# pkhungurn/talking-head-anime-4-demo

Hardware: NVIDIA H100
Metric: 512x512 RGBA frames/sec (higher is better)
Workload: dtype f16/tf32 operands (10-bit mantissa), f32 accumulate, f32 storage outside conv operands

## Files before the change

tha4_b200/csrc/capi.cu:

```cuda
#include "../../include/tha4_b200.h"
#include "nets.cuh"
#include "siren.cuh"
#include "profiler.cuh"
#include "distill.cuh"
#include <atomic>
#include <cstring>
#include <map>
#include <tuple>
#include <vector>

namespace tha4 {
std::atomic<long> g_kernel_launches{0};
bool g_use_pdl = true;
thread_local AllocSink* g_alloc_sink = nullptr;
void* tracked_malloc(size_t bytes) {
    void* p = nullptr;
    THA4_CUDA_CHECK(cudaMalloc(&p, std::max<size_t>(bytes, 16)));
    if (g_alloc_sink) g_alloc_sink->ptrs.push_back(p);
    return p;
}
}

using namespace tha4;

// ... 206 lines not shown
    if (ctx->capture_stream) cudaStreamDestroy(ctx->capture_stream);
    if (ctx->side) { cudaStreamDestroy(ctx->side); cudaEventDestroy(ctx->ev_fork); cudaEventDestroy(ctx->ev_join); }
    if (ctx->stats_base) cudaFree(ctx->stats_base);
    ctx->drop_graphs();
    delete ctx;
    return THA4_OK;
}

const char* tha4_last_error(const tha4_ctx* ctx) { return ctx ? ctx->err.c_str() : g_create_err.c_str(); }

int tha4_set_option(tha4_ctx* ctx, const char* name, int64_t value) {
    return guarded(ctx, [&] {
        cudaDeviceSynchronize();
        ctx->drop_graphs();
        if (!strcmp(name, "strict")) { ctx->strict = value ? 1 : 0; }
        else if (!strcmp(name, "cuda_graphs")) ctx->use_graphs = value ? 1 : 0;
        else if (!strcmp(name, "side_stream")) ctx->side_streams = value ? 1 : 0;
        else if (!strcmp(name, "tcgen05")) conv_enable_tc(value != 0);
        else if (!strcmp(name, "cluster_splitk")) conv_tc_enable_cluster(value != 0);
        else if (!strcmp(name, "halo_conv")) conv_halo_enable(value != 0);
        else if (!strcmp(name, "tma_store")) conv_halo_enable_tma_store(value != 0);
        else if (!strcmp(name, "halo_m256")) { THA4_REQUIRE(value >= -1 && value <= 1, "halo_m256: -1, 0 or 1"); conv_halo_set_m256((int)value); }
        else if (!strcmp(name, "halo_ctas")) { THA4_REQUIRE(value == -1 || value == 1 || value == 2, "halo_ctas: -1, 1 or 2"); conv_halo_set_ctas((int)value); }
        else if (!strcmp(name, "siren_tc")) siren_tc_enable(value != 0);
        else if (!strcmp(name, "tc_stride2")) conv_tc_enable_stride2(value != 0);
        else if (!strcmp(name, "small_bn")) conv_tc_enable_small_bn(value != 0);
        else if (!strcmp(name, "attn_split16")) attention_enable_split16(value != 0);
        else if (!strcmp(name, "tail_persist")) tail_tc_enable_persist(value != 0);
        else if (!strcmp(name, "attn_mma")) attention_enable_mma(value != 0);
        else if (!strcmp(name, "half_operands")) ctx->half_operands = value ? 1 : 0;
        else if (!strcmp(name, "pdl")) g_use_pdl = value != 0;
        else if (!strcmp(name, "profile")) { prof_enable(value != 0); if (value == 2) prof_reset(); }
        else if (!strcmp(name, "microbatch")) { THA4_REQUIRE(value >= 1 && value <= 1024, "microbatch range"); ctx->microbatch = (int)value; }
        else throw std::runtime_error(std::string("tha4: unknown option ") + name);
    });
}

int64_t tha4_get_counter(const tha4_ctx* ctx, const char* name) {
    if (!strcmp(name, "kernel_launches")) return g_kernel_launches.load();
    {
        static const char* cats[] = {"conv", "norm", "tail", "attn", "glue", "siren"};
        static const char* whats[] = {"us", "launches", "flops", "bytes"};
        if (!strncmp(name, "prof_", 5))
            for (int w = 0; w < 4; ++w)
                for (int c = 0; c < 6; ++c)
                    if (std::string(name) == std::string("prof_") + whats[w] + "_" + cats[c]) {
// ... 969 lines not shown
```

tha4_b200/csrc/conv.cuh:

```cuda
#pragma once
#include "common.cuh"

namespace tha4 {

constexpr int CONV_MAX_TAPS = 16;
constexpr int CONV_MAX_PHASES = 4;

enum ResMode { RES_NONE = 0, RES_SAME = 1, RES_UP2 = 2, RES_DOWN2 = 3 };

struct ConvWeights {
    float* w = nullptr;
    mutable __half* w16 = nullptr;
    mutable float w16_scale = 1.0f;
    float* bias = nullptr;
    int cin = 0, cout = 0, cin_pad = 0, cout_pad = 0;
    int ntaps = 0, nphase = 1;
    bool dynamic = false;
    bool tf32_rounded = false;
    int stride = 1;
    int out_mul = 1;
    signed char dy[CONV_MAX_PHASES][CONV_MAX_TAPS];
    signed char dx[CONV_MAX_PHASES][CONV_MAX_TAPS];
    signed char ph_oy[CONV_MAX_PHASES], ph_ox[CONV_MAX_PHASES];
};
// ... 24 lines not shown
    View out16;
    ConvNormIn nin;
    View res;
    int res_mode = RES_NONE;
    int strict = 0;
    int ksplit = 0;
    float* ws = nullptr;
    size_t ws_floats = 0;
};

size_t conv_workspace_floats(const ConvWeights& cw, const ConvArgs& a);

void conv_forward(const ConvWeights& cw, const ConvArgs& a, cudaStream_t s);
void conv_mma_forward(const ConvWeights& cw, const ConvArgs& a, cudaStream_t s);
bool conv_tc_supported(const ConvWeights& cw, const ConvArgs& a);
void conv_tc_forward(const ConvWeights& cw, const ConvArgs& a, cudaStream_t s);
bool conv_fuses_stats(const ConvWeights& cw, const ConvArgs& a);
bool conv_tc_fuses_stats(const ConvWeights& cw, const ConvArgs& a);
bool conv_halo_supported(const ConvWeights& cw, const ConvArgs& a);
void conv_halo_forward(const ConvWeights& cw, const ConvArgs& a, cudaStream_t s);
void conv_halo_enable(bool on);
void conv_halo_enable_tma_store(bool on);
void conv_halo_set_ctas(int mode);
void conv_halo_set_m256(int mode);
void conv_halo_debug_dump();
void conv_enable_tc(bool on);
bool conv_tc_enabled();
void conv_make_half(const ConvWeights& cw, cudaStream_t s);
void conv_tc_enable_cluster(bool on);
void conv_tc_enable_small_bn(bool on);
void conv_tc_enable_stride2(bool on);

}
```

tha4_b200/csrc/conv_halo.cu:

```cuda
#include "conv.cuh"
#include "profiler.cuh"
#include "conv_tc_device.cuh"
#include <cuda.h>
#include <cstring>
#include <map>
#include <mutex>
#include <tuple>

namespace tha4 {
static long long* g_dbg_buf = nullptr;

namespace {

using namespace tc;
using namespace tcdev;

constexpr int HT_W = 8, HT_H = 16;
constexpr int HALO_W = HT_W + 2;
__host__ __device__ constexpr int halo_h(int wg) { return HT_H * wg + 2; }
__host__ __device__ constexpr int halo_rows(int wg) { return HALO_W * halo_h(wg); }
__host__ __device__ constexpr int halo_a_bytes(int rowb, int wg) { return ((halo_rows(wg) * rowb + 1023) / 1024) * 1024; }
__host__ __device__ constexpr int halo_threads(int wg, int ctas = 1) { return 128 * wg + (ctas == 2 ? 0 : 32); }
static_assert((HT_H * HALO_W * 64) % 1024 == 0, "second warpgroup's halo offset keeps the swizzle phase");

__host__ __device__ constexpr int halo_min_ctas(int bn, int sa, int cs, int op, int wg, int ph = 1, int ctas = 1) {
    return ctas == 2 ? 2 : wg > 1 ? (bn * (ph == 4 ? 2 : 1) <= 32 ? 2 : 1) : cs > 1 || bn >= 128 ? 1 : ((sa == (op == OP_F16N ? 2 : 1) && bn <= 32) ? 4 : 2);
}
template <int PH>
__host__ __device__ constexpr int halo_wtile(int j) { return PH == 1 ? j : ((j & 1) * 2 + ((j >> 1) & 1)) * 4 + (j >> 2); }

template <int BN, int SA, int SB, int CS, int OP, int XF, int WG, int PH = 1, int CTAS = 1>
__global__ void __launch_bounds__(halo_threads(WG, CTAS), halo_min_ctas(BN, SA, CS, OP, WG, PH, CTAS)) conv_halo_kernel(const __grid_constant__ CUtensorMap tmA, const __grid_constant__ CUtensorMap tmB,
                                                                const __grid_constant__ CUtensorMap tmO32, const __grid_constant__ CUtensorMap tmO16,
                                                                const __grid_constant__ CUtensorMap tmR, const TcParams p) {
    static_assert(OP != OP_TF32, "halo kernel: f16 operands");
    static_assert(BN <= 128, "the accumulator of one warpgroup: BN registers per thread");
    static_assert(WG == 1 || (WG == 2 && CS == 1 && BN <= 64), "two consumer warpgroups: unsplit launches, two accumulators of at most 64 columns");
    static_assert(PH == 1 || (PH == 4 && WG == 2 && BN <= 32), "four-phase layers: two warpgroups, two 128 x 32 accumulators each");
    constexpr bool SELF_LOAD = CTAS == 2;
    static_assert(CTAS == 1 || (CTAS == 2 && WG == 2), "two CTAs per SM: the two-warpgroup tiles");
    static_assert(!SELF_LOAD || SB >= (PH == 1 ? 3 : 6), "weight ring too shallow for loads issued by a consumer");
    constexpr int SLABS = PH == 1 ? WG : 1;
    constexpr int NACC = PH == 1 ? 1 : 2;
    constexpr int TPC = PH == 1 ? 9 : 16;
    constexpr int ROWB = op_row_bytes(OP);
    constexpr int KCE = op_kch(OP);
    constexpr int HALO_ROWS = halo_rows(SLABS);
    constexpr int A_BYTES = halo_a_bytes(ROWB, SLABS);
    constexpr int B_BYTES = BN * ROWB;
    constexpr int PRODUCER_WARP = 4 * WG;
    constexpr int EPI_BYTES = (int)(((size_t)SA * A_BYTES + (size_t)SB * B_BYTES) / WG) & ~1023;
    constexpr int NSLOT = CS == 1 && PH == 1 ? epi_nslot(BN, EPI_BYTES) : 0;
    extern __shared__ uint8_t smem_raw[];
    uint8_t* smem = smem_raw + ((1024u - (tc::smem_u32(smem_raw) & 1023u)) & 1023u);
    uint8_t* smA = smem;
    uint8_t* smB = smem + SA * A_BYTES;
    uint64_t* bars = reinterpret_cast<uint64_t*>(smB + SB * B_BYTES);
    uint64_t* a_full = bars, *a_empty = bars + SA;
    uint64_t* b_full = bars + 2 * SA, *b_empty = b_full + SB;
    uint64_t* res_bars = b_empty + SB;
    float* xf_A = reinterpret_cast<float*>(reinterpret_cast<uint8_t*>(res_bars + 4 * WG) + ((16u - (tc::smem_u32(res_bars + 4 * WG) & 15u)) & 15u));

    const int warp = threadIdx.x >> 5, lane = threadIdx.x & 31;
    auto dbg_slot = [&]() -> long long* {
        const bool dbg_on = p.dbg != nullptr && (blockIdx.x % 97) == 0 && blockIdx.y == 0 && (blockIdx.x / 97) * CS + blockIdx.z < 32;
        return dbg_on ? p.dbg + ((blockIdx.x / 97) * CS + blockIdx.z) * 32 : nullptr;
    };
    long long* dbg = SELF_LOAD ? nullptr : dbg_slot();
#define HSTAMP(role, i) do { long long* d_ = SELF_LOAD ? dbg_slot() : dbg; if (d_) d_[(role) * 8 + (i)] = clock64(); } while (0)
#define HSTAMP_END(role, i) do { if (!SELF_LOAD) HSTAMP(role, i); } while (0)
    if (threadIdx.x == 0) HSTAMP(0, 0);
    int tile = blockIdx.x;
    const int tx = tile % p.tiles_x; tile /= p.tiles_x;
    const int ty = tile % p.tiles_y;
    const int n = tile / p.tiles_y;
// ... 25 lines not shown
        }
    }
    pdl_wait();
    if (threadIdx.x == 0) HSTAMP(0, 2);

    Acc<BN> acc[NACC];
    if (nc > 0) {
        if (!SELF_LOAD && warp == PRODUCER_WARP) {
            if (lane == 0) {
                int bi = 0;
                for (int ci = 0; ci < nc; ++ci) {
                    const int sa = ci % SA;
                    mbar_wait(smem_u32(a_empty + sa), ((ci / SA) & 1) ^ 1);
                    mbar_expect_tx(smem_u32(a_full + sa), HALO_ROWS * ROWB);
                    tma_load_4d(smem_u32(smA + sa * A_BYTES), &tmA, (cb0 + ci) * KCE, x0 - 1, y0 - 1, n, smem_u32(a_full + sa));
                    for (int tap = 0; tap < TPC; ++tap, ++bi) {
                        if (bi < npre) continue;
                        const int sb = bi % SB;
                        mbar_wait(smem_u32(b_empty + sb), ((bi / SB) & 1) ^ 1);
                        mbar_expect_tx(smem_u32(b_full + sb), B_BYTES);
                        tma_load_3d(smem_u32(smB + sb * B_BYTES), &tmB, (cb0 + ci) * KCE, n0, halo_wtile<PH>(tap), smem_u32(b_full + sb));
                    }
                }
            }
        } else {
            const int te = threadIdx.x;
            const int wg = WG == 1 ? 0 : te >> 7;
            constexpr int XBAR = WG == 1 ? 1 : 3;
            __half* hA = reinterpret_cast<__half*>(xf_A);
            __half* hB = hA + p.xf_C;
            const bool silu = p.xf_act == ACT_SILU || p.xf_act == ACT_SILU_FAST;
            auto load_b = [&](int j) {
                if (j < SB || j >= nb) return;
                const int sb = j % SB;
                mbar_wait(smem_u32(b_empty + sb), ((j / SB) & 1) ^ 1);
                mbar_expect_tx(smem_u32(b_full + sb), B_BYTES);
                tma_load_3d(smem_u32(smB + sb * B_BYTES), &tmB, (cb0 + j / TPC) * KCE, n0, halo_wtile<PH>(j % TPC), smem_u32(b_full + sb));
            };
            auto load_a = [&](int ci) {
                if (ci >= nc) return;
                const int sa = ci % SA;
                mbar_wait(smem_u32(a_empty + sa), ((ci / SA) & 1) ^ 1);
                mbar_expect_tx(smem_u32(a_full + sa), HALO_ROWS * ROWB);
                tma_load_4d(smem_u32(smA + sa * A_BYTES), &tmA, (cb0 + ci) * KCE, x0 - 1, y0 - 1, n, smem_u32(a_full + sa));
            };
            if (SELF_LOAD && te == 0) {
// ... 79 lines not shown
                            Wgmma<BN>::f16(acc[0].d[0], make_desc_sbo<ROWB>(a0 + 32 * k, HALO_W * ROWB), bd, accum);
                            Wgmma<BN>::f16(acc[0].d[1], make_desc_sbo<ROWB>(a1 + 32 * k, HALO_W * ROWB), bd, accum);
                        }
                        wg_commit();
                        if (tap < 8) {
                            wg_wait<1>();
                            if (tap > 0) mbar_arrive(smem_u32(b_empty + (bi - 1) % SB));
                        } else {
                            wg_wait<0>();
                            mbar_arrive(smem_u32(b_empty + (bi - 1) % SB));
                            mbar_arrive(smem_u32(b_empty + bi % SB));
                            mbar_arrive(smem_u32(a_empty + sa));
                        }
                        if (SELF_LOAD && te == 0) {
                            load_b(bi + SB - 2);
                            if (tap == 8) load_a(ci + SA);
                        }
                    }
                }
            }
#pragma unroll
            for (int a = 0; a < NACC; ++a) { wg_fence_acc(acc[a].d[0]); wg_fence_acc(acc[a].d[1]); }
            if (te == 0) { HSTAMP_END(1, 1); HSTAMP_END(2, 3); }
            if constexpr (WG > 1) asm volatile("bar.sync 3, 256;\n" ::: "memory");
            if constexpr (PH == 4) {
#pragma unroll
                for (int px = 0; px < 2; ++px) {
                    if (px > 0) asm volatile("bar.sync 3, 256;\n" ::: "memory");
                    epi_direct<BN, HT_W, 0, WG>(p, acc[px], smem + wg * EPI_BYTES, n, y0, x0, n0, 2 * wg + px, 0, warp, lane,
                                                nullptr, nullptr, nullptr, nullptr, wg, EPI_BYTES);
                }
            } else if (CS == 1) {
                epi_direct<BN, HT_W, NSLOT, WG>(p, acc[0], smem + wg * EPI_BYTES, n, y0 + wg * HT_H, x0, n0, 0, 0, warp, lane,
                                                &tmO32, &tmO16, &tmR, res_bars + 4 * wg, wg, EPI_BYTES);
            }
            if (te == 0) HSTAMP_END(2, 4);
        }
    }
    if (CS > 1) {
        asm volatile("barrier.cluster.arrive.release.aligned;\n" ::: "memory");
        asm volatile("barrier.cluster.wait.acquire.aligned;\n" ::: "memory");
        if (threadIdx.x == 0) HSTAMP(2, 5);
        if (warp < PRODUCER_WARP && nc > 0) epi_push_partial<BN, CS>(acc[0], smem, split, warp, lane);
        asm volatile("barrier.cluster.arrive.release.aligned;\n" ::: "memory");
        asm volatile("barrier.cluster.wait.acquire.aligned;\n" ::: "memory");
        if (threadIdx.x == 0) HSTAMP(2, 7);
        if (warp < PRODUCER_WARP) epi_cluster_reduce<BN, CS, HT_W>(p, smem, n, y0, x0, n0, 0, split, warp, dbg);
        if (threadIdx.x == 0) HSTAMP(2, 6);
    }
    __syncthreads();
    if (threadIdx.x == 0) HSTAMP_END(0, 3);
#undef HSTAMP_END
#undef HSTAMP
}

typedef CUresult (*EncodeTiledFn)(CUtensorMap*, CUtensorMapDataType, cuuint32_t, void*, const cuuint64_t*, const cuuint64_t*,
                                  const cuuint32_t*, const cuuint32_t*, CUtensorMapInterleave, CUtensorMapSwizzle,
                                  CUtensorMapL2promotion, CUtensorMapFloatOOBfill);
EncodeTiledFn halo_encode() {
    static EncodeTiledFn fn = nullptr;
    if (!fn) {
        void* ptr = nullptr;
// ... 47 lines not shown
    const int es = f16 ? 2 : 4;
    if (!v.p || (reinterpret_cast<uintptr_t>(v.p) & 15) || ((long)v.ld * es) % 16 != 0) return false;
    HKey key{current_device(), v.p, v.N, v.H, v.W, v.C, v.ld, f16 ? -2 : -3};
    std::lock_guard<std::mutex> lock(g_halo_mu);
    auto it = g_halo_maps.find(key);
    if (it == g_halo_maps.end()) {
        CUtensorMap m;
        cuuint64_t dims[4] = {(cuuint64_t)v.C, (cuuint64_t)v.W, (cuuint64_t)v.H, (cuuint64_t)v.N};
        cuuint64_t strides[3] = {(cuuint64_t)v.ld * es, (cuuint64_t)v.W * v.ld * es, (cuuint64_t)v.H * v.W * v.ld * es};
        cuuint32_t box[4] = {32, (cuuint32_t)HT_W, (cuuint32_t)HT_H, 1};
        cuuint32_t estr[4] = {1, 1, 1, 1};
        CUresult r = halo_encode()(&m, f16 ? CU_TENSOR_MAP_DATA_TYPE_FLOAT16 : CU_TENSOR_MAP_DATA_TYPE_FLOAT32, 4, v.p, dims, strides, box, estr,
                                   CU_TENSOR_MAP_INTERLEAVE_NONE, f16 ? CU_TENSOR_MAP_SWIZZLE_64B : CU_TENSOR_MAP_SWIZZLE_128B,
                                   CU_TENSOR_MAP_L2_PROMOTION_NONE, CU_TENSOR_MAP_FLOAT_OOB_FILL_NONE);
        if (r != CUDA_SUCCESS) return false;
        it = g_halo_maps.emplace(key, m).first;
    }
    *out = &it->second;
    return true;
}

int g_halo_m256 = -1;
int g_halo_ctas = -1;

constexpr size_t halo_ring(int op, int bn, int sa, int sb, int wg, int ph) {
    return (size_t)sa * halo_a_bytes(op_row_bytes(op), ph == 1 ? wg : 1) + (size_t)sb * bn * op_row_bytes(op);
}
constexpr size_t halo_smem0(int op, int bn, int sa, int sb, int wg, int ph) {
    return 1024 + halo_ring(op, bn, sa, sb, wg, ph) + (2 * sa + 2 * sb + 4 * wg) * 8 + 16;
}

struct HaloPlan { int bn, tiles_x, tiles_y, tiles_m, tiles_n, cs, chunks, wg, ctas; };

constexpr int halo_sb_wg2(int op, int bn, int sa, int sb_min) {
    const size_t a = (size_t)sa * halo_a_bytes(op_row_bytes(op), 2), b = (size_t)bn * op_row_bytes(op);
    int sb = sb_min;
    while (a + sb * b < 2 * (size_t)(epi_slot0(bn) + EPI_SLOT_BYTES)) ++sb;
    return sb;
}
constexpr int halo2_sa(int op, int ph) { return ph == 4 || op == OP_F16N ? 2 : 1; }
constexpr int halo2_sb(int op, int ph) { return ph == 4 ? 12 : halo_sb_wg2(op, 64, halo2_sa(op, ph), op == OP_F16N ? 12 : 6); }

int halo_plan_ctas(int op, int bn, int ph, long ctas, const ConvArgs& a) {
    if (g_halo_ctas > 0) return g_halo_ctas;
    const size_t smem = halo_smem0(op, bn, halo2_sa(op, ph), halo2_sb(op, ph), 2, ph) + (a.nin.on ? (size_t)24 * a.nin.C + 32 : 0);
    return ctas > num_sms() && 2 * (smem + 1024) <= (size_t)228 * 1024 ? 2 : 1;
}

HaloPlan halo_plan(const ConvWeights& cw, const ConvArgs& a, int op) {
    HaloPlan pl;
    pl.chunks = cw.cin_pad / op_kch(op);
    if (cw.nphase == 4) {
        pl.tiles_x = ceil_div(a.in.W, HT_W); pl.tiles_y = ceil_div(a.in.H, HT_H);
        pl.tiles_m = pl.tiles_x * pl.tiles_y * a.in.N;
        pl.bn = 32; pl.tiles_n = cw.cout_pad / 32; pl.cs = 1; pl.wg = 2;
        pl.ctas = halo_plan_ctas(op, 32, 4, (long)pl.tiles_m * pl.tiles_n, a);
        return pl;
    }
    pl.tiles_x = ceil_div(a.out.W, HT_W); pl.tiles_y = ceil_div(a.out.H, HT_H);
    pl.tiles_m = pl.tiles_x * pl.tiles_y * a.in.N;
    pl.bn = (cw.cout_pad % 128 == 0) ? 128 : (cw.cout_pad % 64 == 0 ? 64 : 32);
    const int sms = num_sms();
    pl.cs = 1;
    long ctas = (long)pl.tiles_m * (cw.cout_pad / pl.bn);
    const bool m256 = g_halo_m256 > 0 || (g_halo_m256 < 0 && a.ksplit <= 1 && 8L * pl.tiles_m >= sms);
    if (a.ksplit > 1) {
        while (pl.cs * 2 <= std::min(8, a.ksplit)) pl.cs *= 2;
    } else if (a.ksplit <= 0 && ctas < sms * 13 / 16 && !m256) {
        while (pl.bn > 64 && (long)pl.tiles_m * (cw.cout_pad / pl.bn) < sms && cw.cout_pad % (pl.bn / 2) == 0) pl.bn /= 2;
        ctas = (long)pl.tiles_m * (cw.cout_pad / pl.bn);
        const int want = std::max(2, (int)((3 * sms / 2 + ctas - 1) / ctas));
        while (pl.cs < 8 && pl.cs * 2 <= want && pl.cs * 2 <= pl.chunks) pl.cs *= 2;
        while (pl.bn > 32 && (long)pl.tiles_m * (cw.cout_pad / pl.bn) * pl.cs < 96 && cw.cout_pad % (pl.bn / 2) == 0) pl.bn /= 2;
    }
    while (pl.cs > 1 && (pl.cs > pl.chunks || ceil_div(pl.chunks, ceil_div(pl.chunks, pl.cs)) != pl.cs)) pl.cs /= 2;
    pl.tiles_n = cw.cout_pad / pl.bn;
    pl.wg = 1;
    if (pl.cs == 1 && m256) {
        pl.wg = 2;
        pl.tiles_y = ceil_div(a.out.H, 2 * HT_H);
        pl.tiles_m = pl.tiles_x * pl.tiles_y * a.in.N;
        pl.bn = std::min(pl.bn, 64);
        pl.tiles_n = cw.cout_pad / pl.bn;
    }
    pl.ctas = pl.wg == 2 && pl.bn == 64 ? halo_plan_ctas(op, 64, 1, (long)pl.tiles_m * pl.tiles_n, a) : 1;
    return pl;
}

template <int OP, int BN, int SA, int SB, int CS, int XF, int WG = 1, int PH = 1, int CTAS = 1>
void launch_halo(const CUtensorMap& ma, const CUtensorMap& mb, const CUtensorMap& mo32, const CUtensorMap& mo16, const CUtensorMap& mr, const TcParams& p, dim3 grid, cudaStream_t s) {
    constexpr size_t ring = halo_ring(OP, BN, SA, SB, WG, PH);
    constexpr size_t smem0 = halo_smem0(OP, BN, SA, SB, WG, PH);
    static_assert(smem0 <= 227 * 1024, "shared memory budget");
    static_assert(ring / WG >= (size_t)4 * 32 * 33 * 4 + 4 * BN * 8, "epilogue scratch must fit in the pipeline buffers");
    static_assert(WG == 1 || PH == 4 || epi_nslot(BN, (ring / WG) & ~(size_t)1023) > 0, "two warpgroups: a TMA-store staging slot each");
    static_assert(CS == 1 || ring >= (size_t)128 * BN * 4 + 128 * 8 * 4 + 128 * 4 * 4, "partial tile + statistics scratch must fit");
    static_assert(CTAS == 1 || 2 * (smem0 + 1024) <= 228 * 1024, "two CTAs per SM");
    const size_t smem = smem0 + (XF ? (size_t)24 * p.xf_C + 32 : 0);
    THA4_REQUIRE(smem <= 227 * 1024, "conv_halo: shared memory budget (fused input normalisation)");
    THA4_ENSURE_SMEM((conv_halo_kernel<BN, SA, SB, CS, OP, XF, WG, PH, CTAS>), smem);
    launch_pdl(conv_halo_kernel<BN, SA, SB, CS, OP, XF, WG, PH, CTAS>, grid, dim3(halo_threads(WG, CTAS)), smem, s, CS, ma, mb, mo32, mo16, mr, p);
    THA4_LAUNCH_CHECK();
}

template <int OP, int BN, int SA, int SBD, int SBS, int XF>
void launch_halo_cs(int cs, int wg, int ctas, const CUtensorMap& ma, const CUtensorMap& mb, const CUtensorMap& mo32, const CUtensorMap& mo16, const CUtensorMap& mr, const TcParams& p, dim3 grid, cudaStream_t s) {
    constexpr int SA1 = OP == OP_F16N ? 2 : 1;
    THA4_REQUIRE(wg == 1 || (BN <= 64 && cs == 1), "conv_halo: 256-pixel tiles need an unsplit launch with N tiles of at most 64 columns");
    THA4_REQUIRE(ctas == 1 || (wg == 2 && BN == 64), "conv_halo: two CTAs per SM are built for 256 x 64 tiles");
    if constexpr (BN == 64) {
        if (ctas == 2) {
            launch_halo<OP, 64, halo2_sa(OP, 1), halo2_sb(OP, 1), 1, XF, 2, 1, 2>(ma, mb, mo32, mo16, mr, p, grid, s);
            return;
        }
    }
    if constexpr (BN <= 64) {
        if (cs == 1 && p.cpt == 1) {
            if (wg == 2) launch_halo<OP, BN, SA1, halo_sb_wg2(OP, BN, SA1, BN == 64 ? SBD : SBS), 1, XF, 2>(ma, mb, mo32, mo16, mr, p, grid, s);
            else launch_halo<OP, BN, SA1, SBS, 1, XF>(ma, mb, mo32, mo16, mr, p, grid, s);
            return;
        }
    }
    if constexpr (BN <= 64) {
        if (wg == 2) {
            constexpr int M = OP == OP_F16N ? 2 : 1;
            launch_halo<OP, BN, SA, halo_sb_wg2(OP, BN, SA, BN == 64 ? SBD : 2 * M), 1, XF, 2>(ma, mb, mo32, mo16, mr, p, grid, s);
            return;
        }
    }
    if (cs == 8) launch_halo<OP, BN, SA, SBD, 8, XF>(ma, mb, mo32, mo16, mr, p, grid, s);
    else if (cs == 4) launch_halo<OP, BN, SA, SBD, 4, XF>(ma, mb, mo32, mo16, mr, p, grid, s);
    else if (cs == 2) launch_halo<OP, BN, SA, SBD, 2, XF>(ma, mb, mo32, mo16, mr, p, grid, s);
    else if ((long)grid.x * grid.y * grid.z <= num_sms())
        launch_halo<OP, BN, SA, SBD, 1, XF>(ma, mb, mo32, mo16, mr, p, grid, s);
    else launch_halo<OP, BN, SA, SBS, 1, XF>(ma, mb, mo32, mo16, mr, p, grid, s);
}

template <int OP, int XF>
void launch_halo_bn(int bn, int cs, int wg, int ctas, const CUtensorMap& ma, const CUtensorMap& mb, const CUtensorMap& mo32, const CUtensorMap& mo16, const CUtensorMap& mr, const TcParams& p, dim3 grid, cudaStream_t s) {
    constexpr int M = OP == OP_F16N ? 2 : 1;
    if (bn == 128) launch_halo_cs<OP, 128, 2 * M, 6 * M, 3 * M, XF>(cs, wg, ctas, ma, mb, mo32, mo16, mr, p, grid, s);
    else if (bn == 64) launch_halo_cs<OP, 64, 2 * M, 8 * M, 3 * M, XF>(cs, wg, ctas, ma, mb, mo32, mo16, mr, p, grid, s);
    else launch_halo_cs<OP, 32, 2 * M, 9 * M, 5 * M, XF>(cs, wg, ctas, ma, mb, mo32, mo16, mr, p, grid, s);
}

bool g_use_halo = true;
bool g_tma_store = true;

}

void conv_halo_enable(bool on) { g_use_halo = on; }
void conv_halo_enable_tma_store(bool on) { g_tma_store = on; }
void conv_halo_set_m256(int mode) { g_halo_m256 = mode; }
void conv_halo_set_ctas(int mode) { g_halo_ctas = mode; }

bool conv_halo_supported(const ConvWeights& cw, const ConvArgs& a) {
    if (!g_use_halo || !conv_tc_supported(cw, a)) return false;
    if (!a.in.f16 || cw.stride != 1) return false;
    const bool four_phase = cw.nphase == 4 && cw.ntaps == 4 && cw.out_mul == 2;
    if (!four_phase && (cw.ntaps != 9 || cw.nphase != 1 || cw.out_mul != 1)) return false;
    for (int ph = 0; ph < cw.nphase; ++ph)
        for (int t = 0; t < cw.ntaps; ++t)
            if (cw.dy[ph][t] < -1 || cw.dy[ph][t] > 1 || cw.dx[ph][t] < -1 || cw.dx[ph][t] > 1) return false;
    if (!four_phase) return a.in.H == a.out.H && a.in.W == a.out.W;
    if (cw.cin_pad % 64 != 0 || a.ksplit > 1 || a.out.H != 2 * a.in.H || a.out.W != 2 * a.in.W) return false;
    const HaloPlan pl = halo_plan(cw, a, OP_F16);
    return a.ksplit == 1 || (long)pl.tiles_m * pl.tiles_n >= 64;
}

bool conv_halo_fuses_stats(const ConvWeights&, const ConvArgs&) { return true; }

void conv_halo_forward(const ConvWeights& cw, const ConvArgs& a, cudaStream_t s) {
    THA4_REQUIRE(conv_halo_supported(cw, a), "conv_halo: unsupported configuration");
    THA4_REQUIRE(a.in.C == cw.cin && a.out.C == cw.cout && a.in.N == a.out.N, "conv_halo: shapes");
    const int op = cw.cin_pad % 64 == 0 ? OP_F16 : OP_F16N;
    TcParams p{};
    p.out = a.out.p; p.outH = a.out.H; p.outW = a.out.W; p.outC = a.out.C; p.out_ld = a.out.ld;
// ... 22 lines not shown
    p.acc_scale = 1.0f / cw.w16_scale;
    for (int ph = 0; ph < cw.nphase; ++ph) {
        p.ph_oy[ph] = cw.ph_oy[ph]; p.ph_ox[ph] = cw.ph_ox[ph];
        for (int t = 0; t < cw.ntaps; ++t) { p.dy[ph][t] = cw.dy[ph][t]; p.dx[ph][t] = cw.dx[ph][t]; }
    }
    p.ksplit = 1;
    p.ws = nullptr;
    p.stats = a.out.stats; p.stats_ld = a.out.stats_ld;
    p.stats_rep = std::max(1, a.out.stats_rep); p.stats_rep_stride = a.out.stats_rep_stride;
    static const bool dbg_env = getenv("THA4_HALO_DEBUG") != nullptr;
    if (dbg_env) {
        if (!g_dbg_buf) { THA4_CUDA_CHECK(cudaMalloc(&g_dbg_buf, 32 * 32 * sizeof(long long))); }
        THA4_CUDA_CHECK(cudaMemsetAsync(g_dbg_buf, 0, 32 * 32 * sizeof(long long), s));
        p.dbg = g_dbg_buf;
    }
    ProfScope prof(PROF_CONV, s);
    prof_add_work(PROF_CONV, 2.0 * (double)p.N * p.MH * p.MW * cw.cout * cw.cin * cw.ntaps * cw.nphase, 0.0);
    const CUtensorMap& ma = halo_activation_map(a.in, op, cw.nphase == 1 ? pl.wg : 1);
    const CUtensorMap& mb = halo_weight_map(cw, pl.bn, op);
    const CUtensorMap* mo32 = &ma;
    const CUtensorMap* mo16 = &ma;
    const CUtensorMap* mr = &ma;
    p.st_tma = 0;
    if (pl.cs == 1 && g_tma_store && cw.nphase == 1) {
        if (a.out.p && halo_store_map(a.out, false, &mo32)) p.st_tma |= 1;
        if (a.out16.p && halo_store_map(a.out16, true, &mo16)) p.st_tma |= 2;
        if ((p.st_tma & 1) && a.res.p && p.res_mode == RES_SAME && !a.res.f16 && a.res.N == a.out.N && a.res.H == a.out.H &&
            a.res.W == a.out.W && a.res.C >= a.out.C && halo_store_map(a.res, false, &mr)) p.st_tma |= 4;
    }
    p.vec4 = ((!cw.bias || (reinterpret_cast<uintptr_t>(cw.bias) & 15) == 0) &&
              (!a.res.p || ((reinterpret_cast<uintptr_t>(a.res.p) & 15) == 0 && a.res.ld % 4 == 0))) ? 1 : 0;
    dim3 grid(pl.tiles_m, pl.tiles_n, pl.cs);
    if (cw.nphase == 4) {
        constexpr int SA2 = halo2_sa(OP_F16, 4), SB2 = halo2_sb(OP_F16, 4);
        if (pl.ctas == 2) {
            if (a.nin.on) launch_halo<OP_F16, 32, SA2, SB2, 1, 1, 2, 4, 2>(ma, mb, *mo32, *mo16, *mr, p, grid, s);
            else launch_halo<OP_F16, 32, SA2, SB2, 1, 0, 2, 4, 2>(ma, mb, *mo32, *mo16, *mr, p, grid, s);
        } else if (a.nin.on) launch_halo<OP_F16, 32, 2, 16, 1, 1, 2, 4>(ma, mb, *mo32, *mo16, *mr, p, grid, s);
        else launch_halo<OP_F16, 32, 2, 16, 1, 0, 2, 4>(ma, mb, *mo32, *mo16, *mr, p, grid, s);
    } else if (op == OP_F16) {
        if (a.nin.on) launch_halo_bn<OP_F16, 1>(pl.bn, pl.cs, pl.wg, pl.ctas, ma, mb, *mo32, *mo16, *mr, p, grid, s);
        else launch_halo_bn<OP_F16, 0>(pl.bn, pl.cs, pl.wg, pl.ctas, ma, mb, *mo32, *mo16, *mr, p, grid, s);
    } else {
        if (a.nin.on) launch_halo_bn<OP_F16N, 1>(pl.bn, pl.cs, pl.wg, pl.ctas, ma, mb, *mo32, *mo16, *mr, p, grid, s);
        else launch_halo_bn<OP_F16N, 0>(pl.bn, pl.cs, pl.wg, pl.ctas, ma, mb, *mo32, *mo16, *mr, p, grid, s);
    }
    static const bool dbg_all = dbg_env && !strcmp(getenv("THA4_HALO_DEBUG"), "2");
    if (dbg_all) {
        fprintf(stderr, "halo launch: N %d %dx%d cin %d cout %d | bn %d cs %d wg %d chunks %d grid %d x %d | xf %d groups %d act %d res %d out32 %d out16 %d st_tma %d | phases %d ctas %d\n",
                p.N, p.MH, p.MW, cw.cin, cw.cout, pl.bn, pl.cs, pl.wg, pl.chunks, pl.tiles_m, pl.tiles_n, a.nin.on ? 1 : 0, p.xf_groups, p.xf_act,
                p.res_mode, p.out ? 1 : 0, p.out16 ? 1 : 0, p.st_tma, cw.nphase, pl.ctas);
        conv_halo_debug_dump();
    }
}

void conv_halo_debug_dump() {
    if (!g_dbg_buf) return;
    std::vector<long long> h(32 * 32);
    THA4_CUDA_CHECK(cudaDeviceSynchronize());
    THA4_CUDA_CHECK(cudaMemcpy(h.data(), g_dbg_buf, h.size() * sizeof(long long), cudaMemcpyDeviceToHost));
// ... 11 lines not shown
```

tha4_b200/csrc/conv_tc_device.cuh:

```cuda
#pragma once
#include "conv.cuh"
#include "tc_common.cuh"

namespace tha4 {
namespace tcdev {

using namespace tc;



constexpr int TILE_W = 16, TILE_H = 8;
constexpr int TC_THREADS = 160;
constexpr int TC_PRODUCER_WARP = 4;

template <int BN> struct Acc { float d[2][BN / 2]; };

template <int WG>
__device__ __forceinline__ void wg_bar(int wg) {
    if (WG == 1 || wg == 0) asm volatile("bar.sync 1, 128;\n" ::: "memory");
    else asm volatile("bar.sync 2, 128;\n" ::: "memory");
}

template <int BN, int WG = 1>
__device__ __forceinline__ void acc_rows32(const Acc<BN>& acc, int c0, float* stage, uint32_t (&r)[32], int t, int wg) {
// ... 132 lines not shown
                const uint32_t addr = base + ((L ^ ((L >> 3) & 7u)) << 4) + (uint32_t)(col & 3) * 4u;
                const float v0 = acc.d[h][4 * g + 2 * e], v1 = acc.d[h][4 * g + 2 * e + 1];
                if (owner == split) {
                    asm volatile("st.shared.v2.f32 [%0], {%1, %2};\n" :: "r"(addr), "f"(v0), "f"(v1) : "memory");
                } else {
                    uint32_t remote;
                    asm volatile("mapa.shared::cluster.u32 %0, %1, %2;\n" : "=r"(remote) : "r"(addr), "r"(owner));
                    asm volatile("st.shared::cluster.v2.f32 [%0], {%1, %2};\n" :: "r"(remote), "f"(v0), "f"(v1) : "memory");
                }
            }
}

constexpr int EPI_SLOT_BYTES = 128 * 128 + 128 * 64;
__host__ __device__ constexpr int epi_slot0(int bn) { return (4 * 32 * 33 * 4 + 4 * bn * 8 + 1023) & ~1023; }
__host__ __device__ constexpr int epi_nslot(int bn, size_t ring) {
    return ring < (size_t)epi_slot0(bn) + EPI_SLOT_BYTES ? 0
         : ((int)((ring - epi_slot0(bn)) / EPI_SLOT_BYTES) < bn / 32 ? (int)((ring - epi_slot0(bn)) / EPI_SLOT_BYTES) : bn / 32);
}
__device__ __forceinline__ void tma_store_4d(const CUtensorMap* map, uint32_t src, int c0, int c1, int c2, int c3) {
    asm volatile("cp.async.bulk.tensor.4d.global.shared::cta.bulk_group [%0, {%2, %3, %4, %5}], [%1];\n"
                 :: "l"(map), "r"(src), "r"(c0), "r"(c1), "r"(c2), "r"(c3) : "memory");
}

template <int BN, int TW, int NSLOT = 0, int WG = 1>
__device__ __forceinline__ void epi_direct(const TcParams& p, const Acc<BN>& acc, uint8_t* smem, int n, int y0, int x0,
                                           int n0, int phase, int split, int warp, int lane,
                                           const CUtensorMap* tm32 = nullptr, const CUtensorMap* tm16 = nullptr,
                                           const CUtensorMap* tmR = nullptr, uint64_t* res_bars = nullptr,
                                           int wg = 0, int wg_bytes = 0) {
    static_assert(WG == 1 || WG == 2, "one or two consumer warpgroups");
    const int q = warp & 3;
    const int t = WG == 1 ? (int)threadIdx.x : (int)threadIdx.x & 127;
    const bool rows_in = WG == 1 || y0 < p.MH;
    const bool res_tma = NSLOT > 0 && (p.st_tma & 4) != 0;
    const int nsteps = min(BN / 32, (p.outC - n0 + 31) / 32);
    if (res_tma && t == 0) {
        for (int s = 0; s < NSLOT && s < nsteps; ++s) {
            const uint32_t bar = smem_u32(res_bars + s);
            mbar_expect_tx(bar, 128 * 128);
            tma_load_4d(smem_u32(smem + epi_slot0(BN) + s * EPI_SLOT_BYTES), tmR, n0 + s * 32, x0, y0, n, bar);
        }
    }
    const int row = q * 32 + lane;
    const bool lead = (split == 0);
    float* scratch = reinterpret_cast<float*>(smem) + q * (32 * 33);
    const int my = y0 + row / TW, mx = x0 + row % TW;
    const bool valid = my < p.MH && mx < p.MW;
// ... 127 lines not shown
                asm volatile("cp.async.bulk.commit_group;\n" ::: "memory");
                if (res_tma && step + NSLOT < nsteps) {
                    asm volatile("cp.async.bulk.wait_group.read 0;\n" ::: "memory");
                    const uint32_t bar = smem_u32(res_bars + (NSLOT > 0 ? step % NSLOT : 0));
                    mbar_expect_tx(bar, 128 * 128);
                    tma_load_4d(smem_u32(slot), tmR, n0 + (step + NSLOT) * 32, x0, y0, n, bar);
                }
            }
            ++step;
        }
        if (p.stats && p.ksplit == 1) {
#pragma unroll
            for (int j = 0; j < 32; ++j) scratch[lane * 33 + j] = valid ? v[j] : 0.0f;
            __syncwarp();
            float su = 0.0f, sq = 0.0f;
#pragma unroll 8
            for (int rr = 0; rr < 32; ++rr) { const float t = scratch[rr * 33 + lane]; su += t; sq += t * t; }
            __syncwarp();
            float2* part = reinterpret_cast<float2*>(reinterpret_cast<float*>(smem) + 4 * 32 * 33);
            part[q * BN + c0 + lane] = make_float2(su, sq);
        }
    }
    if (p.stats && p.ksplit == 1) {
        if constexpr (WG == 1) asm volatile("bar.sync 1, 128;\n" ::: "memory");
        else asm volatile("bar.sync 3, 256;\n" ::: "memory");
        const float2* part = reinterpret_cast<const float2*>(reinterpret_cast<float*>(smem - wg * wg_bytes) + 4 * 32 * 33);
        double* base = p.stats + (long)(blockIdx.x % p.stats_rep) * p.stats_rep_stride + ((long)n * p.stats_ld + n0) * 2;
        for (int c = (int)threadIdx.x; c < BN; c += 128 * WG) {
            if (n0 + c >= p.outC) break;
            const float2 a = part[c], b = part[BN + c], cc = part[2 * BN + c], d = part[3 * BN + c];
            if constexpr (WG == 1) {
                atomicAdd(base + 2 * c, (double)a.x + (double)b.x + (double)cc.x + (double)d.x);
                atomicAdd(base + 2 * c + 1, (double)a.y + (double)b.y + (double)cc.y + (double)d.y);
            } else {
                const float2* part1 = part + wg_bytes / (int)sizeof(float2);
                const float2 e = part1[c], f = part1[BN + c], g = part1[2 * BN + c], h = part1[3 * BN + c];
                atomicAdd(base + 2 * c, (double)a.x + (double)b.x + (double)cc.x + (double)d.x + (double)e.x + (double)f.x + (double)g.x + (double)h.x);
                atomicAdd(base + 2 * c + 1, (double)a.y + (double)b.y + (double)cc.y + (double)d.y + (double)e.y + (double)f.y + (double)g.y + (double)h.y);
            }
        }
    }
    if (NSLOT > 0 && st_tma && t == 0) asm volatile("cp.async.bulk.wait_group.read 0;\n" ::: "memory");
}

template <int BN, int CS, int TW>
__device__ __forceinline__ void epi_cluster_reduce(const TcParams& p, uint8_t* smem, int n, int y0, int x0, int n0, int phase, int split, int warp,
                                                   long long* dbg = nullptr) {
    constexpr int SL = BN / CS, SC = SL / 4;
    static_assert(SL >= 4 && 128 % SC == 0, "cluster slice");
    const int te = threadIdx.x;
    const int cc = te % SC;
    const int chunk = split * SC + cc;
    const int col = n0 + chunk * 4;
    const uint32_t p_local = smem_u32(smem);
// ... 133 lines not shown
```

Before: 164.5.

## Add row-owning CTA pair split-K for two-warpgroup halo conv tiles

Adds a cluster-of-two mode for the 256-pixel, two-warpgroup halo conv kernel. Each rank covers half the channel chunks, and each warpgroup pushes the half of the rows it does not own to the peer CTA over distributed shared memory. The owning CTA adds the received partials and runs the epilogue, with the idle ring buffer serving as the receive slot. The mode is chosen by default when ksplit is unset and two CTAs per tile still fit within the SM count, so under-filled layers get more parallelism. The cost is extra cluster barriers and the DSMEM traffic for the partial sums.

```diff
diff --git a/tha4_b200/csrc/capi.cu b/tha4_b200/csrc/capi.cu
--- a/tha4_b200/csrc/capi.cu
+++ b/tha4_b200/csrc/capi.cu
@@ -252,6 +252,7 @@
         else if (!strcmp(name, "tma_store")) conv_halo_enable_tma_store(value != 0);
         else if (!strcmp(name, "halo_m256")) { THA4_REQUIRE(value >= -1 && value <= 1, "halo_m256: -1, 0 or 1"); conv_halo_set_m256((int)value); }
         else if (!strcmp(name, "halo_ctas")) { THA4_REQUIRE(value == -1 || value == 1 || value == 2, "halo_ctas: -1, 1 or 2"); conv_halo_set_ctas((int)value); }
+        else if (!strcmp(name, "halo_cs")) { THA4_REQUIRE(value == -1 || value == 1 || value == 2, "halo_cs: -1, 1 or 2"); conv_halo_set_cs((int)value); }
         else if (!strcmp(name, "siren_tc")) siren_tc_enable(value != 0);
         else if (!strcmp(name, "tc_stride2")) conv_tc_enable_stride2(value != 0);
         else if (!strcmp(name, "small_bn")) conv_tc_enable_small_bn(value != 0);
diff --git a/tha4_b200/csrc/conv.cuh b/tha4_b200/csrc/conv.cuh
--- a/tha4_b200/csrc/conv.cuh
+++ b/tha4_b200/csrc/conv.cuh
@@ -70,6 +70,7 @@
 void conv_halo_enable(bool on);
 void conv_halo_enable_tma_store(bool on);
 void conv_halo_set_ctas(int mode);
+void conv_halo_set_cs(int mode);
 void conv_halo_set_m256(int mode);
 void conv_halo_debug_dump();
 void conv_enable_tc(bool on);
diff --git a/tha4_b200/csrc/conv_halo.cu b/tha4_b200/csrc/conv_halo.cu
--- a/tha4_b200/csrc/conv_halo.cu
+++ b/tha4_b200/csrc/conv_halo.cu
@@ -29,13 +29,46 @@
 template <int PH>
 __host__ __device__ constexpr int halo_wtile(int j) { return PH == 1 ? j : ((j & 1) * 2 + ((j >> 1) & 1)) * 4 + (j >> 2); }
 
+__device__ __forceinline__ void cluster_sync_all() {
+    asm volatile("barrier.cluster.arrive.release.aligned;\n" ::: "memory");
+    asm volatile("barrier.cluster.wait.acquire.aligned;\n" ::: "memory");
+}
+
+template <int BN, int NACC>
+__device__ __forceinline__ void halo_push_rows(const Acc<BN> (&acc)[NACC], uint32_t remote, int t) {
+#pragma unroll
+    for (int a = 0; a < NACC; ++a)
+#pragma unroll
+        for (int h = 0; h < 2; ++h)
+#pragma unroll
+            for (int j = 0; j < BN / 2; j += 4) {
+                const uint32_t addr = remote + (uint32_t)((((a * 2 + h) * (BN / 8) + j / 4) * 128 + t) * 16);
+                asm volatile("st.shared::cluster.v4.f32 [%0], {%1, %2, %3, %4};\n" :: "r"(addr), "f"(acc[a].d[h][j]),
+                             "f"(acc[a].d[h][j + 1]), "f"(acc[a].d[h][j + 2]), "f"(acc[a].d[h][j + 3]) : "memory");
+            }
+}
+template <int BN, int NACC>
+__device__ __forceinline__ void halo_add_rows(Acc<BN> (&acc)[NACC], const uint8_t* recv, int t) {
+#pragma unroll
+    for (int a = 0; a < NACC; ++a)
+#pragma unroll
+        for (int h = 0; h < 2; ++h)
+#pragma unroll
+            for (int j = 0; j < BN / 2; j += 4) {
+                const float4 v = *reinterpret_cast<const float4*>(recv + (((a * 2 + h) * (BN / 8) + j / 4) * 128 + t) * 16);
+                acc[a].d[h][j] += v.x; acc[a].d[h][j + 1] += v.y; acc[a].d[h][j + 2] += v.z; acc[a].d[h][j + 3] += v.w;
+            }
+}
+
 template <int BN, int SA, int SB, int CS, int OP, int XF, int WG, int PH = 1, int CTAS = 1>
 __global__ void __launch_bounds__(halo_threads(WG, CTAS), halo_min_ctas(BN, SA, CS, OP, WG, PH, CTAS)) conv_halo_kernel(const __grid_constant__ CUtensorMap tmA, const __grid_constant__ CUtensorMap tmB,
                                                                 const __grid_constant__ CUtensorMap tmO32, const __grid_constant__ CUtensorMap tmO16,
                                                                 const __grid_constant__ CUtensorMap tmR, const TcParams p) {
     static_assert(OP != OP_TF32, "halo kernel: f16 operands");
     static_assert(BN <= 128, "the accumulator of one warpgroup: BN registers per thread");
-    static_assert(WG == 1 || (WG == 2 && CS == 1 && BN <= 64), "two consumer warpgroups: unsplit launches, two accumulators of at most 64 columns");
+    static_assert(WG == 1 || (WG == 2 && (CS == 1 || (CS == 2 && CTAS == 1)) && BN <= 64),
+                  "two consumer warpgroups: unsplit launches or a row-owning pair, two accumulators of at most 64 columns");
+    constexpr bool ROW_SPLIT = WG == 2 && CS == 2;
     static_assert(PH == 1 || (PH == 4 && WG == 2 && BN <= 32), "four-phase layers: two warpgroups, two 128 x 32 accumulators each");
     constexpr bool SELF_LOAD = CTAS == 2;
     static_assert(CTAS == 1 || (CTAS == 2 && WG == 2), "two CTAs per SM: the two-warpgroup tiles");
@@ -50,7 +83,9 @@
     constexpr int B_BYTES = BN * ROWB;
     constexpr int PRODUCER_WARP = 4 * WG;
     constexpr int EPI_BYTES = (int)(((size_t)SA * A_BYTES + (size_t)SB * B_BYTES) / WG) & ~1023;
-    constexpr int NSLOT = CS == 1 && PH == 1 ? epi_nslot(BN, EPI_BYTES) : 0;
+    constexpr int NSLOT = (CS == 1 || ROW_SPLIT) && PH == 1 ? epi_nslot(BN, EPI_BYTES) : 0;
+    constexpr int RECV_BYTES = NACC * 128 * BN * 4;
+    static_assert(!ROW_SPLIT || (RECV_BYTES <= EPI_BYTES && (PH == 4 || NSLOT > 0)), "row-owning pair: receive slot and staging slot in the idle ring");
     extern __shared__ uint8_t smem_raw[];
     uint8_t* smem = smem_raw + ((1024u - (tc::smem_u32(smem_raw) & 1023u)) & 1023u);
     uint8_t* smA = smem;
@@ -122,6 +157,11 @@
                         tma_load_3d(smem_u32(smB + sb * B_BYTES), &tmB, (cb0 + ci) * KCE, n0, halo_wtile<PH>(tap), smem_u32(b_full + sb));
                     }
                 }
+            }
+            if constexpr (ROW_SPLIT) {
+                __syncwarp();
+                cluster_sync_all();
+                cluster_sync_all();
             }
         } else {
             const int te = threadIdx.x;
@@ -247,22 +287,35 @@
 #pragma unroll
             for (int a = 0; a < NACC; ++a) { wg_fence_acc(acc[a].d[0]); wg_fence_acc(acc[a].d[1]); }
             if (te == 0) { HSTAMP_END(1, 1); HSTAMP_END(2, 3); }
-            if constexpr (WG > 1) asm volatile("bar.sync 3, 256;\n" ::: "memory");
-            if constexpr (PH == 4) {
-#pragma unroll
-                for (int px = 0; px < 2; ++px) {
-                    if (px > 0) asm volatile("bar.sync 3, 256;\n" ::: "memory");
-                    epi_direct<BN, HT_W, 0, WG>(p, acc[px], smem + wg * EPI_BYTES, n, y0, x0, n0, 2 * wg + px, 0, warp, lane,
-                                                nullptr, nullptr, nullptr, nullptr, wg, EPI_BYTES);
+            if constexpr (ROW_SPLIT) {
+                cluster_sync_all();
+                if (wg != split) {
+                    uint32_t remote;
+                    asm volatile("mapa.shared::cluster.u32 %0, %1, %2;\n" : "=r"(remote) : "r"(smem_u32(smem + (1 - wg) * EPI_BYTES)), "r"(wg));
+                    halo_push_rows<BN, NACC>(acc, remote, te & 127);
                 }
-            } else if (CS == 1) {
-                epi_direct<BN, HT_W, NSLOT, WG>(p, acc[0], smem + wg * EPI_BYTES, n, y0 + wg * HT_H, x0, n0, 0, 0, warp, lane,
-                                                &tmO32, &tmO16, &tmR, res_bars + 4 * wg, wg, EPI_BYTES);
+                cluster_sync_all();
+                if (wg == split) halo_add_rows<BN, NACC>(acc, smem + (1 - wg) * EPI_BYTES, te & 127);
+            } else if constexpr (WG > 1) {
+                asm volatile("bar.sync 3, 256;\n" ::: "memory");
+            }
+            if (!ROW_SPLIT || wg == split) {
+                if constexpr (PH == 4) {
+#pragma unroll
+                    for (int px = 0; px < 2; ++px) {
+                        if (px > 0 && !ROW_SPLIT) asm volatile("bar.sync 3, 256;\n" ::: "memory");
+                        epi_direct<BN, HT_W, 0, WG, !ROW_SPLIT>(p, acc[px], smem + wg * EPI_BYTES, n, y0, x0, n0, 2 * wg + px, 0, warp, lane,
+                                                                nullptr, nullptr, nullptr, nullptr, wg, EPI_BYTES);
+                    }
+                } else if (CS == 1 || ROW_SPLIT) {
+                    epi_direct<BN, HT_W, NSLOT, WG, !ROW_SPLIT>(p, acc[0], smem + wg * EPI_BYTES, n, y0 + wg * HT_H, x0, n0, 0, 0, warp, lane,
+                                                                &tmO32, &tmO16, &tmR, res_bars + 4 * wg, wg, EPI_BYTES);
+                }
             }
             if (te == 0) HSTAMP_END(2, 4);
         }
     }
-    if (CS > 1) {
+    if constexpr (CS > 1 && !ROW_SPLIT) {
         asm volatile("barrier.cluster.arrive.release.aligned;\n" ::: "memory");
         asm volatile("barrier.cluster.wait.acquire.aligned;\n" ::: "memory");
         if (threadIdx.x == 0) HSTAMP(2, 5);
@@ -356,6 +409,7 @@
 
 int g_halo_m256 = -1;
 int g_halo_ctas = -1;
+int g_halo_cs = -1;
 
 constexpr size_t halo_ring(int op, int bn, int sa, int sb, int wg, int ph) {
     return (size_t)sa * halo_a_bytes(op_row_bytes(op), ph == 1 ? wg : 1) + (size_t)sb * bn * op_row_bytes(op);
@@ -379,6 +433,11 @@
     if (g_halo_ctas > 0) return g_halo_ctas;
     const size_t smem = halo_smem0(op, bn, halo2_sa(op, ph), halo2_sb(op, ph), 2, ph) + (a.nin.on ? (size_t)24 * a.nin.C + 32 : 0);
     return ctas > num_sms() && 2 * (smem + 1024) <= (size_t)228 * 1024 ? 2 : 1;
+}
+
+int halo_plan_cs(long ctas, int chunks, const ConvArgs& a) {
+    if (g_halo_cs == 1 || chunks < 2) return 1;
+    return g_halo_cs == 2 || (a.ksplit <= 0 && 2 * ctas <= num_sms()) ? 2 : 1;
 }
 
 HaloPlan halo_plan(const ConvWeights& cw, const ConvArgs& a, int op) {
@@ -389,6 +448,7 @@
         pl.tiles_m = pl.tiles_x * pl.tiles_y * a.in.N;
         pl.bn = 32; pl.tiles_n = cw.cout_pad / 32; pl.cs = 1; pl.wg = 2;
         pl.ctas = halo_plan_ctas(op, 32, 4, (long)pl.tiles_m * pl.tiles_n, a);
+        if (pl.ctas == 1) pl.cs = halo_plan_cs((long)pl.tiles_m * pl.tiles_n, pl.chunks, a);
         return pl;
     }
     pl.tiles_x = ceil_div(a.out.W, HT_W); pl.tiles_y = ceil_div(a.out.H, HT_H);
@@ -418,6 +478,7 @@
         pl.tiles_n = cw.cout_pad / pl.bn;
     }
     pl.ctas = pl.wg == 2 && pl.bn == 64 ? halo_plan_ctas(op, 64, 1, (long)pl.tiles_m * pl.tiles_n, a) : 1;
+    if (pl.wg == 2 && pl.ctas == 1) pl.cs = halo_plan_cs((long)pl.tiles_m * pl.tiles_n, pl.chunks, a);
     return pl;
 }
 
@@ -440,8 +501,9 @@
 template <int OP, int BN, int SA, int SBD, int SBS, int XF>
 void launch_halo_cs(int cs, int wg, int ctas, const CUtensorMap& ma, const CUtensorMap& mb, const CUtensorMap& mo32, const CUtensorMap& mo16, const CUtensorMap& mr, const TcParams& p, dim3 grid, cudaStream_t s) {
     constexpr int SA1 = OP == OP_F16N ? 2 : 1;
-    THA4_REQUIRE(wg == 1 || (BN <= 64 && cs == 1), "conv_halo: 256-pixel tiles need an unsplit launch with N tiles of at most 64 columns");
-    THA4_REQUIRE(ctas == 1 || (wg == 2 && BN == 64), "conv_halo: two CTAs per SM are built for 256 x 64 tiles");
+    THA4_REQUIRE(wg == 1 || (BN <= 64 && (cs == 1 || (cs == 2 && ctas == 1 && p.cpt >= 2))),
+                 "conv_halo: 256-pixel tiles need N tiles of at most 64 columns, unsplit or a pair of one-CTA-per-SM ranks with chunks each");
+    THA4_REQUIRE(ctas == 1 || (wg == 2 && BN == 64 && cs == 1), "conv_halo: two CTAs per SM are built for unsplit 256 x 64 tiles");
     if constexpr (BN == 64) {
         if (ctas == 2) {
             launch_halo<OP, 64, halo2_sa(OP, 1), halo2_sb(OP, 1), 1, XF, 2, 1, 2>(ma, mb, mo32, mo16, mr, p, grid, s);
@@ -458,7 +520,9 @@
     if constexpr (BN <= 64) {
         if (wg == 2) {
             constexpr int M = OP == OP_F16N ? 2 : 1;
-            launch_halo<OP, BN, SA, halo_sb_wg2(OP, BN, SA, BN == 64 ? SBD : 2 * M), 1, XF, 2>(ma, mb, mo32, mo16, mr, p, grid, s);
+            constexpr int SB2 = halo_sb_wg2(OP, BN, SA, BN == 64 ? SBD : 2 * M);
+            if (cs == 2) launch_halo<OP, BN, SA, SB2, 2, XF, 2>(ma, mb, mo32, mo16, mr, p, grid, s);
+            else launch_halo<OP, BN, SA, SB2, 1, XF, 2>(ma, mb, mo32, mo16, mr, p, grid, s);
             return;
         }
     }
@@ -487,6 +551,7 @@
 void conv_halo_enable_tma_store(bool on) { g_tma_store = on; }
 void conv_halo_set_m256(int mode) { g_halo_m256 = mode; }
 void conv_halo_set_ctas(int mode) { g_halo_ctas = mode; }
+void conv_halo_set_cs(int mode) { g_halo_cs = mode; }
 
 bool conv_halo_supported(const ConvWeights& cw, const ConvArgs& a) {
     if (!g_use_halo || !conv_tc_supported(cw, a)) return false;
@@ -555,7 +620,7 @@
     const CUtensorMap* mo16 = &ma;
     const CUtensorMap* mr = &ma;
     p.st_tma = 0;
-    if (pl.cs == 1 && g_tma_store && cw.nphase == 1) {
+    if ((pl.cs == 1 || pl.wg == 2) && g_tma_store && cw.nphase == 1) {
         if (a.out.p && halo_store_map(a.out, false, &mo32)) p.st_tma |= 1;
         if (a.out16.p && halo_store_map(a.out16, true, &mo16)) p.st_tma |= 2;
         if ((p.st_tma & 1) && a.res.p && p.res_mode == RES_SAME && !a.res.f16 && a.res.N == a.out.N && a.res.H == a.out.H &&
@@ -569,6 +634,10 @@
         if (pl.ctas == 2) {
             if (a.nin.on) launch_halo<OP_F16, 32, SA2, SB2, 1, 1, 2, 4, 2>(ma, mb, *mo32, *mo16, *mr, p, grid, s);
             else launch_halo<OP_F16, 32, SA2, SB2, 1, 0, 2, 4, 2>(ma, mb, *mo32, *mo16, *mr, p, grid, s);
+        } else if (pl.cs == 2) {
+            THA4_REQUIRE(pl.chunks >= 2, "conv_halo: a row-owning pair needs a channel chunk per rank");
+            if (a.nin.on) launch_halo<OP_F16, 32, 2, 16, 2, 1, 2, 4>(ma, mb, *mo32, *mo16, *mr, p, grid, s);
+            else launch_halo<OP_F16, 32, 2, 16, 2, 0, 2, 4>(ma, mb, *mo32, *mo16, *mr, p, grid, s);
         } else if (a.nin.on) launch_halo<OP_F16, 32, 2, 16, 1, 1, 2, 4>(ma, mb, *mo32, *mo16, *mr, p, grid, s);
         else launch_halo<OP_F16, 32, 2, 16, 1, 0, 2, 4>(ma, mb, *mo32, *mo16, *mr, p, grid, s);
     } else if (op == OP_F16) {
diff --git a/tha4_b200/csrc/conv_tc_device.cuh b/tha4_b200/csrc/conv_tc_device.cuh
--- a/tha4_b200/csrc/conv_tc_device.cuh
+++ b/tha4_b200/csrc/conv_tc_device.cuh
@@ -178,7 +178,7 @@
                  :: "l"(map), "r"(src), "r"(c0), "r"(c1), "r"(c2), "r"(c3) : "memory");
 }
 
-template <int BN, int TW, int NSLOT = 0, int WG = 1>
+template <int BN, int TW, int NSLOT = 0, int WG = 1, bool FOLD = true>
 __device__ __forceinline__ void epi_direct(const TcParams& p, const Acc<BN>& acc, uint8_t* smem, int n, int y0, int x0,
                                            int n0, int phase, int split, int warp, int lane,
                                            const CUtensorMap* tm32 = nullptr, const CUtensorMap* tm16 = nullptr,
@@ -352,14 +352,16 @@
         }
     }
     if (p.stats && p.ksplit == 1) {
+        constexpr bool FOLD2 = WG == 2 && FOLD;
         if constexpr (WG == 1) asm volatile("bar.sync 1, 128;\n" ::: "memory");
-        else asm volatile("bar.sync 3, 256;\n" ::: "memory");
-        const float2* part = reinterpret_cast<const float2*>(reinterpret_cast<float*>(smem - wg * wg_bytes) + 4 * 32 * 33);
+        else if constexpr (FOLD2) asm volatile("bar.sync 3, 256;\n" ::: "memory");
+        else wg_bar<WG>(wg);
+        const float2* part = reinterpret_cast<const float2*>(reinterpret_cast<float*>(smem - (FOLD2 ? wg * wg_bytes : 0)) + 4 * 32 * 33);
         double* base = p.stats + (long)(blockIdx.x % p.stats_rep) * p.stats_rep_stride + ((long)n * p.stats_ld + n0) * 2;
-        for (int c = (int)threadIdx.x; c < BN; c += 128 * WG) {
+        for (int c = FOLD2 ? (int)threadIdx.x : t; c < BN; c += FOLD2 ? 128 * WG : 128) {
             if (n0 + c >= p.outC) break;
             const float2 a = part[c], b = part[BN + c], cc = part[2 * BN + c], d = part[3 * BN + c];
-            if constexpr (WG == 1) {
+            if constexpr (!FOLD2) {
                 atomicAdd(base + 2 * c, (double)a.x + (double)b.x + (double)cc.x + (double)d.x);
                 atomicAdd(base + 2 * c + 1, (double)a.y + (double)b.y + (double)cc.y + (double)d.y);
             } else {
```

After: 170.2, median of 6. 1.03x the previous value.
